# ViV99/slam-experiments

Measured on NVIDIA B200. Metric: hamming_pairs_per_sec, higher is better.
Workload: dtype u8

## Files before the change

slam_experiments_b200/csrc/hm_tc.cu:

```cuda
#include <math.h>
#include <stdlib.h>

#include <mutex>
#include <type_traits>

#include <cuda_fp16.h>

#include "hm_common.cuh"
#include "hm_tcgen05.cuh"

#ifndef HM_F4_TILE_N
#define HM_F4_TILE_N 128
#endif

namespace hm {

namespace {

constexpr int kRowBlock = 128;
constexpr int kMBlocks = 2;
constexpr int kBlockM = kRowBlock * kMBlocks;
constexpr int kSlabBytes = kRowBlock * 128;
constexpr int kPadRows = HM_PREPARED_TILE_ROWS;
constexpr int kTmemCols = 512;
constexpr uint32_t kSpinLimit = 1u << 26;

static_assert(kPadRows % kBlockM == 0, "prepared padding must cover whole query blocks");

struct CoreI8 {
    using Acc = int;
    static constexpr int kSlabs = 2;
    static constexpr int kRowBytes = HM_PREPARED_ROW_BYTES;
    static constexpr int kTileN = 128;
    static constexpr int kStages = 4;
    static constexpr int kUnits = 4;
    static constexpr int kColSplit = 1;
    static constexpr bool kRegisterHandover = false;
    static constexpr bool kScales = false;
    static constexpr int kPrologueTiles = 45;
    static __device__ __forceinline__ Acc lowest() { return INT_MIN; }
    static __device__ __forceinline__ Acc from_bits(uint32_t x) { return (int)x; }
    static __device__ __forceinline__ Acc max3(Acc a, Acc b, Acc c) { return __vimax3_s32(a, b, c); }
    static __device__ __forceinline__ Acc max2(Acc a, Acc b) { return max(a, b); }
    static __device__ __forceinline__ bool valid(Acc v) { return v >= -256; }
    static __device__ __forceinline__ unsigned distance(Acc v) { return (unsigned)((256 - v) >> 1); }
    static __device__ __forceinline__ unsigned encode(Acc v) { return (unsigned)(v + 257); }
    static __device__ __forceinline__ Acc floor_from(unsigned e) { return (int)e - 259; }
    static __device__ __forceinline__ uint32_t pack2(uint32_t lo, uint32_t hi) { return ((uint32_t)max((int)lo, -32768) & 0xFFFFu) | ((uint32_t)max((int)hi, -32768) << 16); }
    static __device__ __forceinline__ Acc unpack(uint32_t p, int hi) { return hi ? (int)p >> 16 : (int)(short)(p & 0xFFFFu); }
    static constexpr uint32_t kLowestBits = 0x80000000u;
};

struct CoreF4 {
    using Acc = float;
    static constexpr int kSlabs = 1;
    static constexpr int kRowBytes = HM_PREPARED_F4_ROW_BYTES;
    static constexpr int kTileN = HM_F4_TILE_N;
#ifndef HM_F4_STAGES
#define HM_F4_STAGES 6
#endif
    static constexpr int kStages = HM_F4_TILE_N == 96 ? 10 : HM_F4_TILE_N == 64 ? 14 : HM_F4_STAGES;
#ifndef HM_F4_UNITS
#define HM_F4_UNITS (HM_F4_TILE_N == 96 ? 5 : HM_F4_TILE_N == 64 ? 7 : 3)
#endif
    static constexpr int kUnits = HM_F4_UNITS;
    static constexpr int kColSplit = 2;
    static constexpr bool kRegisterHandover = true;
    static constexpr bool kScales = true;
    static constexpr int kPrologueTiles = 90;
    static __device__ __forceinline__ Acc lowest() { return -INFINITY; }
    static __device__ __forceinline__ Acc from_bits(uint32_t x) { return __uint_as_float(x); }
    static __device__ __forceinline__ Acc max3(Acc a, Acc b, Acc c) { return fmaxf(fmaxf(a, b), c); }
    static __device__ __forceinline__ Acc max2(Acc a, Acc b) { return fmaxf(a, b); }
    static __device__ __forceinline__ bool valid(Acc v) { return v >= -256.0f; }
    static __device__ __forceinline__ unsigned distance(Acc v) { return (unsigned)((256 - (int)v) >> 1); }
    static __device__ __forceinline__ unsigned encode(Acc v) { return (unsigned)((int)v + 257); }
    static __device__ __forceinline__ Acc floor_from(unsigned e) { return (float)((int)e - 259); }
    static __device__ __forceinline__ uint32_t pack2(uint32_t lo, uint32_t hi)
    {
        const __half2 h = __floats2half2_rn(__uint_as_float(lo), __uint_as_float(hi));
        return *reinterpret_cast<const uint32_t*>(&h);
    }
    static __device__ __forceinline__ Acc unpack(uint32_t p, int hi)
    {
        const __half2 h = *reinterpret_cast<const __half2*>(&p);
        return hi ? __high2float(h) : __low2float(h);
    }
    static constexpr uint32_t kLowestBits = 0xFF800000u;
};

template <class C> __host__ __device__ constexpr int row_block_bytes() { return kRowBlock * C::kRowBytes; }
template <class C> __host__ __device__ constexpr int a_bytes() { return kMBlocks * row_block_bytes<C>(); }
template <class C> __host__ __device__ constexpr int b_stage_bytes() { return C::kTileN * C::kRowBytes; }
template <class C> __host__ __device__ constexpr int epilogue_warps() { return 4 * kMBlocks * C::kColSplit; }
template <class C> __host__ __device__ constexpr int control_warps() { return C::kRegisterHandover ? 4 : 2; }
template <class C> __host__ __device__ constexpr int threads() { return 32 * (control_warps<C>() + epilogue_warps<C>()); }
constexpr int kHandoverBytes = kBlockM * 16;
constexpr int kBarrierBytes = 512;
template <class C> __host__ __device__ constexpr int smem_bytes() { return 1024 + a_bytes<C>() + C::kStages * b_stage_bytes<C>() + kBarrierBytes + kHandoverBytes; }
static_assert((2 * CoreF4::kStages + 1 + 2 * CoreF4::kUnits) * 8 + 16 <= kBarrierBytes, "barrier block");
static_assert((2 * CoreI8::kStages + 1 + 2 * CoreI8::kUnits) * 8 + 16 <= kBarrierBytes, "barrier block");
__host__ __device__ constexpr int ct_gcd(int a, int b) { return b == 0 ? a : ct_gcd(b, a % b); }
template <class C> __host__ __device__ constexpr int issuer_period() { return C::kStages / ct_gcd(C::kStages, C::kUnits) * C::kUnits; }
constexpr int kScaleCols = 32;
constexpr int kScaleCol = kTmemCols - kScaleCols;
static_assert(CoreF4::kUnits * CoreF4::kTileN <= kScaleCol, "accumulator units must end before the scale factors");

struct PrepareParams {
    const uint8_t* bits;
    long long n, stride, batch_stride;
    long long padded_rows;
    uint8_t* out;
};

__global__ void __launch_bounds__(256) hm_prepare_kernel(const PrepareParams P)
{
    const long long chunks_per_problem = P.padded_rows * 16;
    const long long o = (long long)blockIdx.x * blockDim.x + threadIdx.x;
    if (o >= chunks_per_problem) return;
    const int b = blockIdx.y;
    const long long rb = o >> 11;
    const int rem = (int)(o & 2047);
    const int slab = rem >> 10;
    const int rem2 = rem & 1023;
    const int rr = (rem2 >> 3) & 7;
    const int r = ((rem2 >> 6) << 3) | rr;
    const int c = (rem2 & 7) ^ rr;
    const long long row = rb * kRowBlock + r;
    uint4 v = make_uint4(0, 0, 0, 0);
    if (row < P.n) {
        const uint8_t* src = P.bits + (long long)b * P.batch_stride + row * P.stride + slab * 16 + c * 2;
        const unsigned bits16 = (unsigned)src[0] | ((unsigned)src[1] << 8);
        unsigned w[4];
#pragma unroll
        for (int i = 0; i < 4; ++i) {
            const unsigned nib = (bits16 >> (4 * i)) & 0xF;
            const unsigned spread = (nib & 1) | ((nib & 2) << 7) | ((nib & 4) << 14) | ((nib & 8) << 21);
            w[i] = (spread * 0xFEu) ^ 0xFFFFFFFFu;
        }
        v = make_uint4(w[0], w[1], w[2], w[3]);
    }
    uint4* dst = reinterpret_cast<uint4*>(P.out + (long long)b * P.padded_rows * HM_PREPARED_ROW_BYTES);
    dst[o] = v;
}

__device__ __forceinline__ uint4 expand_bits_e2m1(unsigned bits32)
{
    unsigned w[4];
#pragma unroll
    for (int i = 0; i < 4; ++i) {
        const unsigned by = (bits32 >> (8 * i)) & 0xFF;
        unsigned sgn = 0;
#pragma unroll
        for (int j = 0; j < 8; ++j) sgn |= ((by >> j) & 1u) << (4 * j + 3);
        w[i] = 0xAAAAAAAAu ^ sgn;
    }
    return make_uint4(w[0], w[1], w[2], w[3]);
}

__global__ void __launch_bounds__(256) hm_prepare_f4_kernel(const PrepareParams P)
{
    const long long chunks_per_problem = P.padded_rows * 8;
    const long long o = (long long)blockIdx.x * blockDim.x + threadIdx.x;
    if (o >= chunks_per_problem) return;
    const int b = blockIdx.y;
    const long long rb = o >> 10;
    const int rem = (int)(o & 1023);
    const int rr = (rem >> 3) & 7;
    const int r = ((rem >> 6) << 3) | rr;
    const int c = (rem & 7) ^ rr;
    const long long row = rb * kRowBlock + r;
    uint4 v = make_uint4(0, 0, 0, 0);
    if (row < P.n) {
        const unsigned bits32 = *reinterpret_cast<const unsigned*>(P.bits + (long long)b * P.batch_stride + row * P.stride + c * 4);
        v = expand_bits_e2m1(bits32);
    }
    uint4* dst = reinterpret_cast<uint4*>(P.out + (long long)b * P.padded_rows * HM_PREPARED_F4_ROW_BYTES);
    dst[o] = v;
}

struct TcParams {
    const uint8_t* qbits;
    long long q_bits_stride, q_bits_batch_stride;
    const int* q_index;
    long long q_index_batch_stride;
    const int* nq_dyn;
    const uint8_t* qprep;
    const uint8_t* tprep;
    long long nq, nt;
    long long q_padded, t_padded;
    int tiles_per_split;
    int ntiles;
    unsigned long long train_base;
    unsigned long long* out;
    long long out_split_stride;
    int* error_flag;
    unsigned long long* final_out;
    unsigned* counters;
    int splits;
    unsigned* row_floor;
    ExchangeArgs xch;
    long long q_blocks_valid;
    long long* clock_probe;
    SelectArgs sel;
    long long* trace;
    int trace_first;
};

#ifndef HM_TC_TRACE
#define HM_TC_TRACE 0
#endif
#ifndef HM_TC_EXPERIMENT
#define HM_TC_EXPERIMENT 0
#endif
#ifndef HM_ISSUER_LAST
#define HM_ISSUER_LAST 1
#endif
constexpr bool kIssuerLast = HM_ISSUER_LAST != 0;
#ifndef HM_COMMIT_MODE
#define HM_COMMIT_MODE 0
#endif
constexpr int kTraceTiles = 96;
constexpr int kTraceSlots = 8;
constexpr int kCtaSlots = 24;
__device__ __forceinline__ void cta_mark(const TcParams& P, int slot)
{
#if HM_TC_TRACE
    if (P.trace) {
        unsigned long long t;
        asm volatile("mov.u64 %0, %%globaltimer;" : "=l"(t));
        const long long cta = ((long long)blockIdx.z * gridDim.y + blockIdx.y) * gridDim.x + blockIdx.x;
        long long* rec = P.trace + kTraceTiles * kTraceSlots + cta * kCtaSlots;
        rec[slot] = (long long)t;
        rec[slot + 12] = clock64();
        if (slot == 0) {
            unsigned smid;
            asm volatile("mov.u32 %0, %%smid;" : "=r"(smid));
            rec[11] = smid;
        }
    }
#endif
}
__device__ __forceinline__ void trace_mark(const TcParams& P, int tile, int slot)
{
#if HM_TC_TRACE == 1
    tile -= P.trace_first;
    if (P.trace && blockIdx.x == 0 && blockIdx.y == 0 && blockIdx.z == 0 && tile >= 0 && tile < kTraceTiles)
        P.trace[tile * kTraceSlots + slot] = clock64();
#endif
}

template <class Acc>
struct Top2 {
    Acc v1, v2;
    unsigned i1, i2;
    uint32_t sa[4], sb[4];
    Acc f;
#if HM_TC_TRACE
    unsigned slow;
#endif
};

__device__ __forceinline__ void bounded_wait(uint64_t* bar, uint32_t parity, int* error_flag)
{
    uint32_t spins = 0;
    while (!ptx::mbar_try_wait(bar, parity)) {
        if (++spins > kSpinLimit) {
            if (error_flag) atomicExch(error_flag, 1);
            __trap();
        }
    }
}

__device__ __forceinline__ void bounded_wait_addr(uint32_t bar_addr, uint32_t parity, int* error_flag)
{
    uint32_t spins = 0;
    while (!ptx::mbar_try_wait_addr(bar_addr, parity)) {
        if (++spins > kSpinLimit) {
            if (error_flag) atomicExch(error_flag, 1);
            __trap();
        }
    }
}

#define HM_R8(a, o) "+r"(a[o]), "+r"(a[o + 1]), "+r"(a[o + 2]), "+r"(a[o + 3]), "+r"(a[o + 4]), "+r"(a[o + 5]), "+r"(a[o + 6]), "+r"(a[o + 7])
#define HM_R32(a) HM_R8(a, 0), HM_R8(a, 8), HM_R8(a, 16), HM_R8(a, 24)
__device__ __forceinline__ void tmem_ld_fence4(uint32_t (&a)[32], uint32_t (&b)[32], uint32_t (&c)[32], uint32_t (&d)[32])
{
    asm volatile("tcgen05.wait::ld.sync.aligned;\n" : HM_R32(a), HM_R32(b), HM_R32(c), HM_R32(d) : : "memory");
}
__device__ __forceinline__ void tmem_ld_fence48(uint32_t (&a)[32], uint32_t (&b)[16])
{
    asm volatile("tcgen05.wait::ld.sync.aligned;\n" : HM_R32(a), HM_R8(b, 0), HM_R8(b, 8) : : "memory");
}
__device__ __forceinline__ void tmem_ld_fence64(uint32_t (&a)[64])
{
    asm volatile("tcgen05.wait::ld.sync.aligned;\n" : HM_R8(a, 0), HM_R8(a, 8), HM_R8(a, 16), HM_R8(a, 24), HM_R8(a, 32), HM_R8(a, 40), HM_R8(a, 48), HM_R8(a, 56) : : "memory");
}

template <class C, int kMode, int kGroups = 4>
__device__ __forceinline__ void scan_chunk(const uint32_t* r, unsigned colbase, Top2<typename C::Acc>& s)
{
    using Acc = typename C::Acc;
    static_assert(kGroups == 2 || kGroups == 4 || kGroups == 8, "8-column groups per compare");
    Acc gm[kGroups];
#pragma unroll
    for (int g = 0; g < kGroups; ++g) {
        const int o = g * 8;
        gm[g] = C::max3(C::max3(C::from_bits(r[o]), C::from_bits(r[o + 1]), C::from_bits(r[o + 2])),
                        C::max3(C::from_bits(r[o + 3]), C::from_bits(r[o + 4]), C::from_bits(r[o + 5])),
                        C::max2(C::from_bits(r[o + 6]), C::from_bits(r[o + 7])));
    }
    Acc m;
    if constexpr (kGroups == 8) m = C::max3(C::max3(gm[0], gm[1], gm[2]), C::max3(gm[3], gm[4], gm[5]), C::max2(gm[6], gm[7]));
    else if constexpr (kGroups == 4) m = C::max3(gm[0], gm[1], C::max2(gm[2], gm[3]));
    else m = C::max2(gm[0], gm[1]);
    constexpr bool kFloor = kMode == 1, kTop1 = kMode == 2;
    if (m > (kFloor ? s.f : kTop1 ? s.v1 : s.v2)) {
#if HM_TC_TRACE
        s.slow += 1;
#endif
#pragma unroll
        for (int g = 0; g < kGroups; ++g) {
            const Acc x = gm[g];
            if (x > (kFloor ? s.f : kTop1 ? s.v1 : s.v2)) {
                const int o = g * 8;
                const uint32_t p0 = C::pack2(r[o], r[o + 1]), p1 = C::pack2(r[o + 2], r[o + 3]);
                const uint32_t p2 = C::pack2(r[o + 4], r[o + 5]), p3 = C::pack2(r[o + 6], r[o + 7]);
                const unsigned idx = colbase + o;
                if (kTop1 || x > s.v1) {
                    if (!kTop1) {
                        s.v2 = s.v1; s.i2 = s.i1;
                        s.sb[0] = s.sa[0]; s.sb[1] = s.sa[1]; s.sb[2] = s.sa[2]; s.sb[3] = s.sa[3];
                    }
                    s.v1 = x; s.i1 = idx;
                    s.sa[0] = p0; s.sa[1] = p1; s.sa[2] = p2; s.sa[3] = p3;
                } else {
                    s.v2 = x; s.i2 = idx;
                    s.sb[0] = p0; s.sb[1] = p1; s.sb[2] = p2; s.sb[3] = p3;
                }
                if (kFloor) s.f = C::max2(s.v2, s.f);
            }
        }
    }
}

template <class C, int kN>
__device__ __forceinline__ void mask_tail(uint32_t* r, unsigned colbase, unsigned limit)
{
    if (colbase + kN > limit) {
#pragma unroll
        for (int j = 0; j < kN; ++j)
            if (colbase + j >= limit) r[j] = C::kLowestBits;
    }
}

#ifndef HM_ARRIVE_ELECT
#define HM_ARRIVE_ELECT 1
#endif
#ifndef HM_SCAN_FLAT64
#define HM_SCAN_FLAT64 1
#endif
#ifndef HM_FLOOR_DENSE_TILES
#define HM_FLOOR_DENSE_TILES 32
#endif
#ifndef HM_FLOOR_LATE_MASK
#define HM_FLOOR_LATE_MASK 15
#endif

#ifndef HM_F4_A_TMEM
#define HM_F4_A_TMEM 0
#endif
constexpr int kATmemCol = 384;
constexpr int kATmemColsPerBlock = 32;

template <class C>
__device__ __forceinline__ void issue_half(int h, uint32_t a_block, uint32_t b_stage, uint32_t tmem_d, uint32_t idesc,
                                           uint32_t tmem_sf)
{
    constexpr int kHalf = C::kSlabs * 2;
#pragma unroll
    for (int jj = 0; jj < kHalf; ++jj) {
        const int j = h * kHalf + jj;
        const int slab = j >> 2, k = j & 3;
        const uint64_t db = ptx::kmajor_sw128_desc_from_lo(b_stage + ((slab * kSlabBytes + k * 32) >> 4));
        if constexpr (C::kScales && HM_F4_A_TMEM) {
            ptx::mma_mxf4_ts(tmem_d, a_block + 8 * j, db, idesc, tmem_sf, tmem_sf + kScaleCols / 2, j != 0);
        } else {
            const uint64_t da = ptx::kmajor_sw128_desc_from_lo(a_block + ((slab * kSlabBytes + k * 32) >> 4));
            if constexpr (C::kScales) ptx::mma_mxf4_ss(tmem_d, da, db, idesc, tmem_sf, tmem_sf + kScaleCols / 2, j != 0);
            else                      ptx::mma_i8_ss(tmem_d, da, db, idesc, j != 0);
        }
    }
}

template <class C, int kMode>
__device__ __forceinline__ void tc_knn2_body(const TcParams& P)
{
    constexpr bool kFloor = kMode == 1;
    using Acc = typename C::Acc;
    constexpr int kStages = C::kStages;
    constexpr int kUnits = C::kUnits;
    constexpr int kABytes = a_bytes<C>();
    constexpr int kBStageBytes = b_stage_bytes<C>();
    constexpr int kRowBlockBytes = row_block_bytes<C>();
    constexpr int kTileN = C::kTileN;

    extern __shared__ uint8_t smem_raw[];
    uint8_t* smem = smem_raw + ((1024u - (ptx::smem_u32(smem_raw) & 1023u)) & 1023u);
    uint8_t* smem_a = smem;
    uint8_t* smem_b = smem + kABytes;
    uint64_t* bars = reinterpret_cast<uint64_t*>(smem + kABytes + kStages * kBStageBytes);
    uint64_t* full_bar = bars;
    uint64_t* empty_bar = bars + kStages;
    uint64_t* a_full_bar = bars + 2 * kStages;
    uint64_t* tmem_full_bar = bars + 2 * kStages + 1;
    uint64_t* tmem_empty_bar = tmem_full_bar + kUnits;
    uint32_t* tmem_base_slot = reinterpret_cast<uint32_t*>(tmem_empty_bar + kUnits);
    uint32_t* smem_base_slot = tmem_base_slot + 2;
    ulonglong2* handover = reinterpret_cast<ulonglong2*>(smem + kABytes + kStages * kBStageBytes + kBarrierBytes);

    const int warp = __shfl_sync(0xffffffffu, threadIdx.x >> 5, 0);
    const int lane = threadIdx.x & 31;
    if (threadIdx.x == 0) cta_mark(P, 0);
    if (threadIdx.x == 0 && (blockIdx.x | blockIdx.y | blockIdx.z) == 0 && P.clock_probe) {
        unsigned long long t;
        asm volatile("mov.u64 %0, %%globaltimer;" : "=l"(t));
        P.clock_probe[0] = (long long)t;
        P.clock_probe[1] = clock64();
    }
    const int qb = blockIdx.x;
    const int split = blockIdx.y;
    const int b = blockIdx.z;

    const uint32_t cs = ptx::cluster_nctarank();
    const uint32_t crank = ptx::cluster_ctarank();
    const uint16_t cmask = (uint16_t)((1u << cs) - 1);
    const bool has_a = qb < P.q_blocks_valid;
    auto rows_present = [&]() -> long long { return P.nq_dyn ? min((long long)__ldg(P.nq_dyn + b), P.nq) : P.nq; };
    if (P.nq_dyn && (long long)(qb - (int)crank) * kBlockM >= rows_present()) return;

    const int tile_begin = split * P.tiles_per_split;
    const int tile_end = min(tile_begin + P.tiles_per_split, P.ntiles);
    const int my_tiles = tile_end - tile_begin;

    constexpr int kProducerWarp = kIssuerLast ? epilogue_warps<C>() : 0;
    constexpr int kIssuerWarp = kIssuerLast ? epilogue_warps<C>() + 1 : 1;
    constexpr int kFirstEpiWarp = kIssuerLast ? 0 : 2;
    static_assert(kIssuerLast || !C::kRegisterHandover, "the control warps must form the last warpgroup");
    static_assert(!C::kRegisterHandover || (epilogue_warps<C>() == 16 && threads<C>() == 640),
                  "the register budget (4 x 32 + 16 x 112 = 20 x 96) assumes 20 warps launched at 96 registers");
    if (warp == kProducerWarp && lane == 0) {
        *smem_base_slot = ptx::smem_u32(smem);
        for (int i = 0; i < kStages; ++i) {
            ptx::mbar_init(&full_bar[i], 1);
            ptx::mbar_init(&empty_bar[i], cs);
        }
        ptx::mbar_init(a_full_bar, 1);
        for (int i = 0; i < kUnits; ++i) {
            ptx::mbar_init(&tmem_full_bar[i], 1);
            ptx::mbar_init(&tmem_empty_bar[i], 4 * C::kColSplit);
        }
        ptx::fence_barrier_init();
        ptx::fence_proxy_async();
    } else if (warp == kIssuerWarp) {
        ptx::tmem_alloc(tmem_base_slot, kTmemCols);
        ptx::tmem_relinquish();
    }
    ptx::tc_fence_before();
    if (cs > 1) ptx::cluster_sync();
    else __syncthreads();
    ptx::tc_fence_after();
    const uint32_t tmem_base = *tmem_base_slot;

    if constexpr (C::kScales) {
        if (warp >= kFirstEpiWarp && warp < kFirstEpiWarp + 4) {
            uint32_t ones[32];
#pragma unroll
            for (int i = 0; i < 32; ++i) ones[i] = 0x7F7F7F7Fu;
            const uint32_t taddr = tmem_base + ((uint32_t)((warp & 3) * 32) << 16) + kScaleCol;
            static_assert(kScaleCols == 32, "one x32 store per lane quarter");
            ptx::tmem_st_32x32(taddr, ones);
            ptx::tmem_st_wait();
        }
        if (HM_F4_A_TMEM) {
            static_assert(!HM_F4_A_TMEM || C::kUnits * C::kTileN <= kATmemCol, "accumulator units overlap the A operand");
            static_assert(!HM_F4_A_TMEM || kATmemCol + kMBlocks * kATmemColsPerBlock <= kScaleCol, "A operand overlaps the scale factors");
            if (warp >= kFirstEpiWarp && warp < kFirstEpiWarp + 4 * kMBlocks) {
                const int wq = warp & 3, wblk = ((warp - kFirstEpiWarp) >> 2) & 1;
                const int r = wq * 32 + lane;
                const long long qrow = (long long)qb * kBlockM + wblk * kRowBlock + r;
                uint32_t words[32];
#pragma unroll
                for (int i = 0; i < 32; ++i) words[i] = 0u;
                if (qrow < rows_present()) {
                    if (P.qbits) {
                        const int* qidx = P.q_index ? P.q_index + (long long)b * P.q_index_batch_stride : nullptr;
                        const long long srow = qidx ? (long long)__ldg(qidx + qrow) : qrow;
                        const uint4* src = reinterpret_cast<const uint4*>(P.qbits + (long long)b * P.q_bits_batch_stride + srow * P.q_bits_stride);
                        const uint4 lo = src[0], hi = src[1];
                        const unsigned bits[8] = {lo.x, lo.y, lo.z, lo.w, hi.x, hi.y, hi.z, hi.w};
#pragma unroll
                        for (int c = 0; c < 8; ++c) {
                            const uint4 v = expand_bits_e2m1(bits[c]);
                            words[4 * c] = v.x; words[4 * c + 1] = v.y; words[4 * c + 2] = v.z; words[4 * c + 3] = v.w;
                        }
                    } else if (has_a) {
                        const uint8_t* img = P.qprep + ((long long)b * P.q_padded + (long long)qb * kBlockM + wblk * kRowBlock) * C::kRowBytes;
                        const uint4* row = reinterpret_cast<const uint4*>(img + (r >> 3) * 1024 + (r & 7) * 128);
#pragma unroll
                        for (int c = 0; c < 8; ++c) {
                            const uint4 v = row[c ^ (r & 7)];
                            words[4 * c] = v.x; words[4 * c + 1] = v.y; words[4 * c + 2] = v.z; words[4 * c + 3] = v.w;
                        }
                    }
                }
                ptx::tmem_st_32x32(tmem_base + ((uint32_t)(wq * 32) << 16) + kATmemCol + wblk * kATmemColsPerBlock, words);
                ptx::tmem_st_wait();
            }
        } else if (P.qbits) {
            const uint8_t* qsrc = P.qbits + (long long)b * P.q_bits_batch_stride;
            const int* qidx = P.q_index ? P.q_index + (long long)b * P.q_index_batch_stride : nullptr;
            const long long nq_eff = rows_present();
            for (int o = threadIdx.x; o < kBlockM * 8; o += blockDim.x) {
                const int blk = o >> 10, rem = o & 1023;
                const int rr = (rem >> 3) & 7;
                const int r = ((rem >> 6) << 3) | rr;
                const int c = (rem & 7) ^ rr;
                const long long qrow = (long long)qb * kBlockM + blk * kRowBlock + r;
                uint4 v = make_uint4(0, 0, 0, 0);
                if (qrow < nq_eff) {
                    const long long srow = qidx ? (long long)__ldg(qidx + qrow) : qrow;
                    v = expand_bits_e2m1(*reinterpret_cast<const unsigned*>(qsrc + srow * P.q_bits_stride + c * 4));
                }
                reinterpret_cast<uint4*>(smem_a)[o] = v;
            }
            ptx::fence_proxy_async();
        }
        ptx::tc_fence_before();
        __syncthreads();
        ptx::tc_fence_after();
    }

    if (threadIdx.x == 0) cta_mark(P, 1);
    ulonglong2 my_keys = make_ulonglong2(kNoMatch, kNoMatch);
    long long my_row = -1;
    int my_row_in_cta = 0;

    auto run_producer = [&]() {
        if (lane == 0) {
            if (has_a && !P.qbits && !(C::kScales && HM_F4_A_TMEM)) {
                const uint8_t* qsrc = P.qprep + ((long long)b * P.q_padded + (long long)qb * kBlockM) * C::kRowBytes;
                ptx::mbar_arrive_expect_tx(a_full_bar, kABytes);
                ptx::bulk_g2s(smem_a, qsrc, kABytes, a_full_bar);
            }
            const uint8_t* tsrc = P.tprep + (long long)b * P.t_padded * C::kRowBytes;
            const uint32_t piece = kBStageBytes / cs;
            for (int i = 0; i < (HM_TC_EXPERIMENT >= 5 ? 0 : my_tiles); ++i) {
                const int stage = i % kStages;
                const uint32_t use = i / kStages;
#if HM_TC_EXPERIMENT < 4
                bounded_wait(&empty_bar[stage], (use & 1) ^ 1, P.error_flag);
#endif
                trace_mark(P, i, 0);
                ptx::mbar_arrive_expect_tx(&full_bar[stage], kBStageBytes);
                uint8_t* dst = smem_b + stage * kBStageBytes + crank * piece;
                const uint8_t* src = tsrc + (long long)(tile_begin + i) * kBStageBytes + crank * piece;
                if (cs > 1) ptx::bulk_g2s_multicast(dst, src, piece, &full_bar[stage], cmask);
                else        ptx::bulk_g2s(dst, src, piece, &full_bar[stage]);
            }
        }
    };
    auto run_issuer = [&]() {
        const bool leader = ptx::elect_one();
        const uint32_t idesc = C::kScales ? ptx::make_mxf4_idesc(kRowBlock, kTileN) : ptx::make_i8_idesc(kRowBlock, kTileN);
        constexpr bool kATmem = C::kScales && HM_F4_A_TMEM;
        const uint32_t a_addr = kATmem ? tmem_base + kATmemCol : ptx::smem_u32(smem_a) >> 4;
        constexpr uint32_t kABlockStep = kATmem ? (uint32_t)kATmemColsPerBlock : (uint32_t)(kRowBlockBytes >> 4);
        const uint32_t b_addr = ptx::smem_u32(smem_b) >> 4;
        const uint32_t tmem_sf = tmem_base + kScaleCol;
        if (has_a && !P.qbits && !(C::kScales && HM_F4_A_TMEM)) bounded_wait(a_full_bar, 0, P.error_flag);
        constexpr int kPeriod = issuer_period<C>();
        static_assert(kPeriod % kStages == 0 && (2 * kPeriod) % kUnits == 0 && ((2 * kPeriod / kUnits) & 1) == 0,
                      "unit parities must repeat with the period");
        uint32_t sphase = 0;
        bool ready0 = false;
        for (int base = 0; base < my_tiles; base += kPeriod) {
#pragma unroll
            for (int j = 0; j < kPeriod; ++j) {
                if (base + j < my_tiles) {
                    const int stage = j % kStages;
                    const uint32_t full_par = sphase ^ ((j / kStages) & 1);
                    const int unit_a = (2 * j) % kUnits, unit_b = (2 * j + 1) % kUnits;
                    const uint32_t par_a = (((2 * j) / kUnits) & 1) ^ 1, par_b = (((2 * j + 1) / kUnits) & 1) ^ 1;
                    const uint32_t b_stage = b_addr + stage * (kBStageBytes >> 4);
                    if (leader) trace_mark(P, base + j, 7);
                    if (!ready0) {
#if HM_TC_EXPERIMENT < 4
                        bounded_wait(&full_bar[stage], full_par, P.error_flag);
#endif
#if HM_TC_EXPERIMENT < 3
                        bounded_wait(&tmem_empty_bar[unit_a], par_a, P.error_flag);
#endif
                    }
                    if (leader) trace_mark(P, base + j, 1);
                    ptx::tc_fence_after();
                    if (leader) issue_half<C>(0, a_addr, b_stage, tmem_base + unit_a * kTileN, idesc, tmem_sf);
#if HM_TC_EXPERIMENT >= 3
                    const bool ready1 = true;
#else
                    const bool ready1 = __all_sync(0xffffffffu, ptx::mbar_test_wait(&tmem_empty_bar[unit_b], par_b));
#endif
                    if (leader) {
                        issue_half<C>(1, a_addr, b_stage, tmem_base + unit_a * kTileN, idesc, tmem_sf);
#if HM_TC_EXPERIMENT != 6 && HM_COMMIT_MODE == 0
                        ptx::tc_commit(&tmem_full_bar[unit_a]);
#endif
                    }
                    if (!ready1) bounded_wait(&tmem_empty_bar[unit_b], par_b, P.error_flag);
                    if (leader) trace_mark(P, base + j, 6);
                    ptx::tc_fence_after();
                    if (leader) issue_half<C>(0, a_addr + kABlockStep, b_stage, tmem_base + unit_b * kTileN, idesc, tmem_sf);
                    ready0 = false;
                    if (base + j + 1 < my_tiles) {
                        const int n = j + 1;
#if HM_TC_EXPERIMENT >= 4
                        ready0 = true;
#else
                        ready0 = __all_sync(0xffffffffu,
                                            ptx::mbar_test_wait(&full_bar[n % kStages], sphase ^ ((n / kStages) & 1))
#if HM_TC_EXPERIMENT < 3
                                            && ptx::mbar_test_wait(&tmem_empty_bar[(2 * n) % kUnits], (((2 * n) / kUnits) & 1) ^ 1)
#endif
                                            );
#endif
                    }
                    if (leader) {
                        issue_half<C>(1, a_addr + kABlockStep, b_stage, tmem_base + unit_b * kTileN, idesc, tmem_sf);
#if HM_TC_EXPERIMENT == 6 || HM_COMMIT_MODE == 1
                        ptx::tc_commit(&tmem_full_bar[unit_a]);
#endif
                        ptx::tc_commit(&tmem_full_bar[unit_b]);
                        if (cs > 1) ptx::tc_commit_multicast(&empty_bar[stage], cmask);
                        else        ptx::tc_commit(&empty_bar[stage]);
                    }
                }
            }
            sphase ^= (kPeriod / kStages) & 1;
        }
        __syncwarp();
    };
    auto run_epilogue = [&]() {
        constexpr int kCols = kTileN / C::kColSplit;
        const int quarter = warp & 3;
        const int mblk = ((warp - kFirstEpiWarp) >> 2) & 1;
        const int half = (warp - kFirstEpiWarp) >> 3;
        const int row_in_cta = mblk * kRowBlock + quarter * 32 + lane;
        const long long row = (long long)qb * kBlockM + row_in_cta;
        Top2<Acc> s;
        s.v1 = s.v2 = C::lowest();
        s.i1 = s.i2 = 0;
#pragma unroll
        for (int e = 0; e < 4; ++e) s.sa[e] = s.sb[e] = 0;
        s.f = C::floor_from(0);
#if HM_TC_TRACE
        s.slow = 0;
#endif
        unsigned floor_code = 0;
        const long long first_row = (long long)tile_begin * kTileN;
        const unsigned limit = (unsigned)min((long long)my_tiles * kTileN, P.nt - first_row);
        const uint32_t bars_addr = ptx::lds_volatile_u32(ptx::smem_u32(smem_base_slot)) + kABytes + kStages * kBStageBytes;
        const uint32_t unit_full_addr = bars_addr + (2 * kStages + 1) * 8;
        const uint32_t unit_empty_addr = unit_full_addr + kUnits * 8;
        int unit = mblk;
        uint32_t unit_use = 0;
        unsigned floor_pending = 0;
        auto refresh_floor = [&](int i) {
            if constexpr (kFloor) {
                if (i < HM_FLOOR_DENSE_TILES || (i & HM_FLOOR_LATE_MASK) == 0) {
                    floor_code = max(floor_code, floor_pending);
                    s.f = C::max2(s.f, C::floor_from(floor_code));
                    if (row < P.nq) {
                        unsigned* floor_ptr = P.row_floor + ((long long)b * P.nq + row);
                        const unsigned e = C::valid(s.v2) ? C::encode(s.v2) : 0u;
                        if (e > floor_code) { atomicMax(floor_ptr, e); floor_code = e; }
                        floor_pending = __ldcg(floor_ptr);
                    }
                }
            }
        };
        auto process_tile = [&](int i) {
            bounded_wait_addr(unit_full_addr + unit * 8, unit_use & 1, P.error_flag);
#if HM_TC_TRACE == 2
            if (warp == kFirstEpiWarp && lane == 0 && (i == 8 || i == 32 || i == 64 || i == 192)) cta_mark(P, i == 8 ? 5 : i == 32 ? 6 : i == 64 ? 7 : 8);
#endif
            if (warp == kFirstEpiWarp && lane == 0) trace_mark(P, i, 3);
            if (warp == kFirstEpiWarp + 7 && lane == 0) trace_mark(P, i, 5);
            ptx::tc_fence_after();
            const uint32_t taddr = tmem_base + ((uint32_t)(quarter * 32) << 16) + unit * kTileN + half * kCols;
            const unsigned colbase = (unsigned)i * kTileN + half * kCols;
            if constexpr (C::kColSplit == 1) {
                uint32_t r0[32], r1[32], r2[32], r3[32];
                ptx::tmem_ld_32x32(taddr, r0);
                ptx::tmem_ld_32x32(taddr + 32, r1);
                ptx::tmem_ld_32x32(taddr + 64, r2);
                ptx::tmem_ld_32x32(taddr + 96, r3);
                refresh_floor(i);
                tmem_ld_fence4(r0, r1, r2, r3);
                ptx::tc_fence_before();
                __syncwarp();
                if (HM_ARRIVE_ELECT ? ptx::elect_one() : lane == 0) ptx::mbar_arrive_addr(unit_empty_addr + unit * 8);
                if (colbase + kCols > limit) {
                    mask_tail<C, 32>(r0, colbase, limit);
                    mask_tail<C, 32>(r1, colbase + 32, limit);
                    mask_tail<C, 32>(r2, colbase + 64, limit);
                    mask_tail<C, 32>(r3, colbase + 96, limit);
                }
                scan_chunk<C, kMode>(r0, colbase, s);
                scan_chunk<C, kMode>(r1, colbase + 32, s);
                scan_chunk<C, kMode>(r2, colbase + 64, s);
                scan_chunk<C, kMode>(r3, colbase + 96, s);
            } else {
                if constexpr (kCols == 64) {
                    uint32_t r[64];
#if HM_TC_EXPERIMENT < 2
                    ptx::tmem_ld_32x64(taddr, r);
                    refresh_floor(i);
                    tmem_ld_fence64(r);
#endif
                    ptx::tc_fence_before();
                    __syncwarp();
                    if (HM_ARRIVE_ELECT ? ptx::elect_one() : lane == 0) ptx::mbar_arrive_addr(unit_empty_addr + unit * 8);
#if HM_TC_EXPERIMENT != 0
                    unit += 2;
                    if (unit >= kUnits) { unit -= kUnits; ++unit_use; }
                    return;
#endif
                    mask_tail<C, 64>(r, colbase, limit);
#if HM_SCAN_FLAT64
                    scan_chunk<C, kMode, 8>(r, colbase, s);
#else
                    scan_chunk<C, kMode>(r, colbase, s);
                    scan_chunk<C, kMode>(r + 32, colbase + 32, s);
#endif
                } else if constexpr (kCols == 32) {
                    uint32_t r[32];
                    ptx::tmem_ld_32x32(taddr, r);
                    refresh_floor(i);
                    asm volatile("tcgen05.wait::ld.sync.aligned;\n" : HM_R32(r) : : "memory");
                    ptx::tc_fence_before();
                    __syncwarp();
                    if (HM_ARRIVE_ELECT ? ptx::elect_one() : lane == 0) ptx::mbar_arrive_addr(unit_empty_addr + unit * 8);
                    mask_tail<C, 32>(r, colbase, limit);
                    scan_chunk<C, kMode>(r, colbase, s);
                } else {
                    static_assert(kCols == 64 || kCols == 48, "column split");
                    uint32_t r0[32], r1[16];
                    ptx::tmem_ld_32x32(taddr, r0);
                    ptx::tmem_ld_32x16(taddr + 32, r1);
                    refresh_floor(i);
                    tmem_ld_fence48(r0, r1);
                    ptx::tc_fence_before();
                    __syncwarp();
                    if (HM_ARRIVE_ELECT ? ptx::elect_one() : lane == 0) ptx::mbar_arrive_addr(unit_empty_addr + unit * 8);
                    mask_tail<C, 32>(r0, colbase, limit);
                    mask_tail<C, 16>(r1, colbase + 32, limit);
                    scan_chunk<C, kMode>(r0, colbase, s);
                    scan_chunk<C, kMode, 2>(r1, colbase + 32, s);
                }
            }
            unit += 2;
            if (unit >= kUnits) { unit -= kUnits; ++unit_use; }
            if (warp == kFirstEpiWarp && lane == 0) trace_mark(P, i, 4);
        };
#pragma unroll 1
        for (int i = 0; i < my_tiles; ++i) process_tile(i);
        if (warp == kFirstEpiWarp && lane == 0) cta_mark(P, 2);
#if HM_TC_TRACE
        if (P.trace) {
            const long long cta = ((long long)blockIdx.z * gridDim.y + blockIdx.y) * gridDim.x + blockIdx.x;
            long long* rec = P.trace + kTraceTiles * kTraceSlots + cta * kCtaSlots;
            const unsigned any = __reduce_max_sync(0xffffffffu, s.slow);
            const unsigned sum = __reduce_add_sync(0xffffffffu, s.slow);
            if (lane == 0) { atomicAdd((unsigned long long*)&rec[9], (unsigned long long)any); atomicAdd((unsigned long long*)&rec[10], (unsigned long long)sum); }
        }
#endif
        const unsigned long long gbase = P.train_base + (unsigned long long)first_row;
        auto fold_group = [&](Acc v, unsigned i0, const uint32_t (&p)[4]) {
            if (!C::valid(v)) return;
#pragma unroll
            for (int e = 0; e < 8; ++e) {
                const Acc x = C::unpack(p[e >> 1], e & 1);
                if (C::valid(x)) top2_insert(my_keys.x, my_keys.y, ((unsigned long long)C::distance(x) << 32) | (gbase + i0 + e));
            }
        };
        fold_group(s.v1, s.i1, s.sa);
        if (kMode != 2) fold_group(s.v2, s.i2, s.sb);
        else my_keys.y = kNoMatch;
        if (half == 1) handover[row_in_cta] = my_keys;
        else my_row = row;
        my_row_in_cta = row_in_cta;
    };

    auto run_tail = [&](auto worker_tag) {
        constexpr bool kWorker = decltype(worker_tag)::value;
        ptx::tc_fence_before();
        if (cs > 1) ptx::cluster_sync();
        else __syncthreads();
        if (kWorker && threadIdx.x == 0) cta_mark(P, 3);
        if (warp == kIssuerWarp) {
            ptx::tc_fence_after();
            ptx::tmem_dealloc(tmem_base, kTmemCols);
        }
        if (kWorker && my_row >= 0 && my_row < rows_present()) {
            if constexpr (C::kColSplit == 2) {
                const ulonglong2 o = handover[my_row_in_cta];
                top2_insert(my_keys.x, my_keys.y, o.x);
                top2_insert(my_keys.x, my_keys.y, o.y);
            }
            unsigned long long* out = P.out + (long long)split * P.out_split_stride + ((long long)b * P.nq + my_row) * 2;
            *reinterpret_cast<ulonglong2*>(out) = my_keys;
            if (!P.counters) select_candidate(P.sel, b, my_keys);
        }
        if (P.counters) {
            int* flag = reinterpret_cast<int*>(tmem_base_slot + 1);
            if (last_cta_arrives(&P.counters[(long long)b * gridDim.x + qb], (unsigned)P.splits, flag)) {
                const long long row = (long long)qb * kBlockM + threadIdx.x;
                const bool has_row = kWorker && threadIdx.x < kBlockM && row < rows_present();
                ulonglong2 k = make_ulonglong2(kNoMatch, kNoMatch);
                if (has_row) fold_partials(P.out, P.splits, P.out_split_stride, (long long)b * P.nq + row, k.x, k.y);
                if (P.xch.world > 1 && (long long)qb * kBlockM < P.nq) k = exchange_and_merge(P.xch, row, has_row, k, qb);
                if (has_row) {
                    *reinterpret_cast<ulonglong2*>(P.final_out + ((long long)b * P.nq + row) * 2) = k;
                    select_candidate(P.sel, b, k);
                }
            }
        }
        if (kWorker && threadIdx.x == 0) cta_mark(P, 4);
        if (kWorker && threadIdx.x == 0 && (blockIdx.x | blockIdx.y | blockIdx.z) == 0 && P.clock_probe) {
            unsigned long long t;
            asm volatile("mov.u64 %0, %%globaltimer;" : "=l"(t));
            P.clock_probe[2] = (long long)t;
            P.clock_probe[3] = clock64();
        }
    };

    if constexpr (C::kRegisterHandover) {
        if (warp >= kProducerWarp) {
            asm volatile("setmaxnreg.dec.sync.aligned.u32 32;\n");
            if (warp == kProducerWarp) run_producer();
            else if (warp == kIssuerWarp) run_issuer();
            run_tail(std::false_type{});
            return;
        }
        asm volatile("setmaxnreg.inc.sync.aligned.u32 112;\n");
        run_epilogue();
        run_tail(std::true_type{});
    } else {
        if (warp == kProducerWarp) run_producer();
        else if (warp == kIssuerWarp) run_issuer();
        else run_epilogue();
        run_tail(std::true_type{});
    }
}

__global__ void __launch_bounds__(threads<CoreI8>(), 1) hm_i8_knn2_kernel(const TcParams P) { tc_knn2_body<CoreI8, 0>(P); }
__global__ void __launch_bounds__(threads<CoreF4>(), 1) hm_f4_knn2_kernel(const TcParams P) { tc_knn2_body<CoreF4, 0>(P); }
__global__ void __launch_bounds__(threads<CoreI8>(), 1) hm_i8_knn2_floor_kernel(const TcParams P) { tc_knn2_body<CoreI8, 1>(P); }
__global__ void __launch_bounds__(threads<CoreF4>(), 1) hm_f4_knn2_floor_kernel(const TcParams P) { tc_knn2_body<CoreF4, 1>(P); }
__global__ void __launch_bounds__(threads<CoreI8>(), 1) hm_i8_knn1_kernel(const TcParams P) { tc_knn2_body<CoreI8, 2>(P); }
__global__ void __launch_bounds__(threads<CoreF4>(), 1) hm_f4_knn1_kernel(const TcParams P) { tc_knn2_body<CoreF4, 2>(P); }

using KernelFn = void (*)(const TcParams);
template <class C> KernelFn kernel_of(int mode = 0);
template <> KernelFn kernel_of<CoreI8>(int mode) { return mode == 1 ? hm_i8_knn2_floor_kernel : mode == 2 ? hm_i8_knn1_kernel : hm_i8_knn2_kernel; }
template <> KernelFn kernel_of<CoreF4>(int mode) { return mode == 1 ? hm_f4_knn2_floor_kernel : mode == 2 ? hm_f4_knn1_kernel : hm_f4_knn2_kernel; }

struct TcPlan {
    int ntiles, splits, tiles_per_split;
    int cluster;
    long long qblocks;
};

int floor_max_tiles()
{
    static int v = -1;
    if (v < 0) {
        const char* e = getenv("HM_FLOOR_MAX_TILES");
        v = e ? atoi(e) : 0x7fffffff;
    }
    return v;
}

int floor_min_tiles_unsplit()
{
    static int v = -1;
    if (v < 0) {
        const char* e = getenv("HM_FLOOR_MIN_TILES_UNSPLIT");
        v = e ? atoi(e) : 0x7fffffff;
    }
    return v;
}

int cluster_override()
{
    static int v = -1;
    if (v < 0) {
        const char* e = getenv("HM_I8_CLUSTER");
        v = e ? atoi(e) : 0;
        if (v != 1 && v != 2 && v != 4) v = 0;
    }
    return v;
}

constexpr int kMaxDevices = 64;
std::mutex g_launch_state_mu;

int current_device_slot()
{
    int dev = 0;
    if (cudaGetDevice(&dev) != cudaSuccess) { cudaGetLastError(); dev = 0; }
    return (dev >= 0 && dev < kMaxDevices) ? dev : -1;
}

template <class C>
cudaError_t ensure_smem_opt_in()
{
    static bool done[kMaxDevices] = {};
    const int dev = current_device_slot();
    std::lock_guard<std::mutex> lock(g_launch_state_mu);
    if (dev >= 0 && done[dev]) return cudaSuccess;
    for (int mode = 0; mode < 3; ++mode) {
        const cudaError_t e = cudaFuncSetAttribute(kernel_of<C>(mode), cudaFuncAttributeMaxDynamicSharedMemorySize, smem_bytes<C>());
        if (e != cudaSuccess) return e;
    }
    if (dev >= 0) done[dev] = true;
    return cudaSuccess;
}

template <class C>
int resident_ctas(int cs, int sm_count)
{
    static int cache[kMaxDevices][5] = {};
    if (cs <= 1) return sm_count;
    const int dev = current_device_slot();
    if (dev >= 0) {
        std::lock_guard<std::mutex> lock(g_launch_state_mu);
        if (cache[dev][cs]) return cache[dev][cs];
    }
    int v = sm_count;
    if (ensure_smem_opt_in<C>() == cudaSuccess) {
        cudaLaunchConfig_t cfg{};
        cfg.gridDim = dim3(cs * 64, 1, 1);
        cfg.blockDim = dim3(threads<C>());
        cfg.dynamicSmemBytes = smem_bytes<C>();
        cudaLaunchAttribute attr[1];
        attr[0].id = cudaLaunchAttributeClusterDimension;
        attr[0].val.clusterDim.x = (unsigned)cs;
        attr[0].val.clusterDim.y = 1;
        attr[0].val.clusterDim.z = 1;
        cfg.attrs = attr;
        cfg.numAttrs = 1;
        int n = 0;
        if (cudaOccupancyMaxActiveClusters(&n, kernel_of<C>(), &cfg) == cudaSuccess && n > 0) v = n * cs;
        else cudaGetLastError();
    } else {
        cudaGetLastError();
    }
    if (dev >= 0) {
        std::lock_guard<std::mutex> lock(g_launch_state_mu);
        cache[dev][cs] = v;
    }
    return v;
}

template <class C>
int prologue_tiles()
{
    static int v = -1;
    if (v < 0) {
        const char* e = getenv("HM_PROLOGUE_TILES");
        v = e ? atoi(e) : C::kPrologueTiles;
    }
    return v;
}

int cluster_min_tiles()
{
    static int v = -1;
    if (v < 0) {
        const char* e = getenv("HM_CLUSTER_MIN_TILES");
        v = e ? atoi(e) : 1024;
    }
    return v;
}

template <class C>
TcPlan plan_tc_cluster(long long nq, long long nt, int batch, int sm_count, int cluster)
{
    TcPlan pl{};
    const long long qb = ceil_div(nq, kBlockM);
    pl.cluster = cluster;
    pl.qblocks = ceil_div(qb, pl.cluster) * pl.cluster;
    sm_count = resident_ctas<C>(pl.cluster, sm_count);
    pl.ntiles = (int)ceil_div(nt, C::kTileN);
    const long long items = pl.qblocks * batch;
    long long best_cost = -1;
    int best = 1;
    const int max_splits = (int)min((long long)pl.ntiles, 4096ll);
    for (int s = 1; s <= max_splits; ++s) {
        const long long tps = ceil_div(pl.ntiles, s);
        const long long real_s = ceil_div(pl.ntiles, tps);
        const long long waves = ceil_div(items * real_s, sm_count);
        const long long cost = waves * (tps + prologue_tiles<C>());
        if (best_cost < 0 || cost < best_cost) {
            best_cost = cost;
            best = s;
        }
        if (items * s > 16ll * sm_count) break;
    }
    pl.tiles_per_split = (int)ceil_div(pl.ntiles, best);
    pl.splits = (int)ceil_div(pl.ntiles, pl.tiles_per_split);
    return pl;
}

template <class C>
TcPlan plan_tc(long long nq, long long nt, int batch, int sm_count)
{
    if (cluster_override()) return plan_tc_cluster<C>(nq, nt, batch, sm_count, cluster_override());
    if (ceil_div(nq, kBlockM) >= 2) {
        const TcPlan pl = plan_tc_cluster<C>(nq, nt, batch, sm_count, 2);
        if (pl.tiles_per_split >= cluster_min_tiles()) return pl;
    }
    return plan_tc_cluster<C>(nq, nt, batch, sm_count, 1);
}

template <class C>
long long padded_rows(long long n) { return ceil_div(ceil_div(n, C::kTileN) * C::kTileN, kPadRows) * kPadRows; }

template <class C>
size_t partials_bytes(long long nq, long long nt, int batch, int sm_count)
{
    const TcPlan pl = plan_tc<C>(nq, nt, batch, sm_count);
    return (size_t)pl.splits * batch * nq * 2 * sizeof(unsigned long long);
}

inline size_t zeroed_bytes(long long row_blocks, long long rows) { return counters_bytes(row_blocks) + counters_bytes((rows + 1) / 2 * 2); }

template <class C>
size_t workspace_bytes_of(long long nq, long long nt, int batch, int sm_count, bool with_prepare)
{
    size_t b = 256 + zeroed_bytes(plan_tc<C>(nq, nt, batch, sm_count).qblocks * batch, nq * batch) + partials_bytes<C>(nq, nt, batch, sm_count);
    b = (b + 1023) & ~(size_t)1023;
    if (with_prepare) b += (size_t)(padded_rows<C>(nq) + padded_rows<C>(nt)) * C::kRowBytes * batch;
    return b;
}

template <class C>
int launch_prepared(const void* qprep, long long nq, const void* tprep, long long nt, int batch,
                    unsigned long long train_base, unsigned long long* out, void* ws, size_t ws_bytes,
                    int sm_count, cudaStream_t stream, const unsigned long long** out_partials,
                    int* out_groups, const ExchangeArgs* exchange, bool top1 = false, const QueryBits* qbits = nullptr,
                    const SelectArgs* select = nullptr)
{
    HM_CUDA_CHECK(ensure_smem_opt_in<C>());
    const TcPlan pl = plan_tc<C>(nq, nt, batch, sm_count);
    if ((long long)pl.ntiles * C::kTileN > (1ll << 32)) {
        set_error("train set too large for 32-bit trainIdx");
        return HM_ERR_UNSUPPORTED;
    }
    const bool keep_partials = out == nullptr;
    const size_t cbytes = zeroed_bytes(pl.qblocks * batch, nq * batch);
    const size_t need = 256 + cbytes + partials_bytes<C>(nq, nt, batch, sm_count);
    if (!ws || ws_bytes < need) {
        set_error("workspace too small: need %zu bytes, got %zu", need, ws_bytes);
        return HM_ERR_WORKSPACE;
    }
    TcParams P{};
    if (qbits && qbits->bits) {
// ... 289 lines not shown
```

Before: 13900.

## Unroll epilogue steady state over TMEM units and use three-input max

```diff
diff --git a/slam_experiments_b200/csrc/hm_tc.cu b/slam_experiments_b200/csrc/hm_tc.cu
--- a/slam_experiments_b200/csrc/hm_tc.cu
+++ b/slam_experiments_b200/csrc/hm_tc.cu
@@ -70,7 +70,12 @@
     static constexpr int kPrologueTiles = 90;
     static __device__ __forceinline__ Acc lowest() { return -INFINITY; }
     static __device__ __forceinline__ Acc from_bits(uint32_t x) { return __uint_as_float(x); }
-    static __device__ __forceinline__ Acc max3(Acc a, Acc b, Acc c) { return fmaxf(fmaxf(a, b), c); }
+    static __device__ __forceinline__ Acc max3(Acc a, Acc b, Acc c)
+    {
+        float d;
+        asm("max.f32 %0, %1, %2, %3;" : "=f"(d) : "f"(a), "f"(b), "f"(c));
+        return d;
+    }
     static __device__ __forceinline__ Acc max2(Acc a, Acc b) { return fmaxf(a, b); }
     static __device__ __forceinline__ bool valid(Acc v) { return v >= -256.0f; }
     static __device__ __forceinline__ unsigned distance(Acc v) { return (unsigned)((256 - (int)v) >> 1); }
@@ -298,23 +303,35 @@
     asm volatile("tcgen05.wait::ld.sync.aligned;\n" : HM_R8(a, 0), HM_R8(a, 8), HM_R8(a, 16), HM_R8(a, 24), HM_R8(a, 32), HM_R8(a, 40), HM_R8(a, 48), HM_R8(a, 56) : : "memory");
 }
 
+template <class C, int N>
+__device__ __forceinline__ typename C::Acc max_tree(const typename C::Acc (&v)[N])
+{
+    if constexpr (N == 1) return v[0];
+    else if constexpr (N == 2) return C::max2(v[0], v[1]);
+    else {
+        typename C::Acc w[N / 3 + N % 3];
+#pragma unroll
+        for (int k = 0; k < N / 3; ++k) w[k] = C::max3(v[3 * k], v[3 * k + 1], v[3 * k + 2]);
+#pragma unroll
+        for (int k = 0; k < N % 3; ++k) w[N / 3 + k] = v[3 * (N / 3) + k];
+        return max_tree<C, N / 3 + N % 3>(w);
+    }
+}
+
 template <class C, int kMode, int kGroups = 4>
 __device__ __forceinline__ void scan_chunk(const uint32_t* r, unsigned colbase, Top2<typename C::Acc>& s)
 {
     using Acc = typename C::Acc;
     static_assert(kGroups == 2 || kGroups == 4 || kGroups == 8, "8-column groups per compare");
-    Acc gm[kGroups];
+    Acc part[2 * kGroups];
 #pragma unroll
     for (int g = 0; g < kGroups; ++g) {
         const int o = g * 8;
-        gm[g] = C::max3(C::max3(C::from_bits(r[o]), C::from_bits(r[o + 1]), C::from_bits(r[o + 2])),
-                        C::max3(C::from_bits(r[o + 3]), C::from_bits(r[o + 4]), C::from_bits(r[o + 5])),
-                        C::max2(C::from_bits(r[o + 6]), C::from_bits(r[o + 7])));
-    }
-    Acc m;
-    if constexpr (kGroups == 8) m = C::max3(C::max3(gm[0], gm[1], gm[2]), C::max3(gm[3], gm[4], gm[5]), C::max2(gm[6], gm[7]));
-    else if constexpr (kGroups == 4) m = C::max3(gm[0], gm[1], C::max2(gm[2], gm[3]));
-    else m = C::max2(gm[0], gm[1]);
+        part[2 * g] = C::max3(C::from_bits(r[o]), C::from_bits(r[o + 1]), C::from_bits(r[o + 2]));
+        part[2 * g + 1] = C::max3(C::max3(C::from_bits(r[o + 3]), C::from_bits(r[o + 4]), C::from_bits(r[o + 5])),
+                                  C::from_bits(r[o + 6]), C::from_bits(r[o + 7]));
+    }
+    const Acc m = max_tree<C, 2 * kGroups>(part);
     constexpr bool kFloor = kMode == 1, kTop1 = kMode == 2;
     if (m > (kFloor ? s.f : kTop1 ? s.v1 : s.v2)) {
 #if HM_TC_TRACE
@@ -322,7 +339,7 @@
 #endif
 #pragma unroll
         for (int g = 0; g < kGroups; ++g) {
-            const Acc x = gm[g];
+            const Acc x = C::max2(part[2 * g], part[2 * g + 1]);
             if (x > (kFloor ? s.f : kTop1 ? s.v1 : s.v2)) {
                 const int o = g * 8;
                 const uint32_t p0 = C::pack2(r[o], r[o + 1]), p1 = C::pack2(r[o + 2], r[o + 3]);
@@ -357,9 +374,6 @@
 
 #ifndef HM_ARRIVE_ELECT
 #define HM_ARRIVE_ELECT 1
-#endif
-#ifndef HM_SCAN_FLAT64
-#define HM_SCAN_FLAT64 1
 #endif
 #ifndef HM_FLOOR_DENSE_TILES
 #define HM_FLOOR_DENSE_TILES 32
@@ -672,32 +686,36 @@
         const uint32_t bars_addr = ptx::lds_volatile_u32(ptx::smem_u32(smem_base_slot)) + kABytes + kStages * kBStageBytes;
         const uint32_t unit_full_addr = bars_addr + (2 * kStages + 1) * 8;
         const uint32_t unit_empty_addr = unit_full_addr + kUnits * 8;
-        int unit = mblk;
-        uint32_t unit_use = 0;
+        const uint32_t tmem_warp = tmem_base + ((uint32_t)(quarter * 32) << 16) + half * kCols;
         unsigned floor_pending = 0;
-        auto refresh_floor = [&](int i) {
+        auto refresh_floor = [&]() {
             if constexpr (kFloor) {
-                if (i < HM_FLOOR_DENSE_TILES || (i & HM_FLOOR_LATE_MASK) == 0) {
-                    floor_code = max(floor_code, floor_pending);
-                    s.f = C::max2(s.f, C::floor_from(floor_code));
-                    if (row < P.nq) {
-                        unsigned* floor_ptr = P.row_floor + ((long long)b * P.nq + row);
-                        const unsigned e = C::valid(s.v2) ? C::encode(s.v2) : 0u;
-                        if (e > floor_code) { atomicMax(floor_ptr, e); floor_code = e; }
-                        floor_pending = __ldcg(floor_ptr);
-                    }
+                floor_code = max(floor_code, floor_pending);
+                s.f = C::max2(s.f, C::floor_from(floor_code));
+                if (row < P.nq) {
+                    unsigned* floor_ptr = P.row_floor + ((long long)b * P.nq + row);
+                    const unsigned e = C::valid(s.v2) ? C::encode(s.v2) : 0u;
+                    if (e > floor_code) { atomicMax(floor_ptr, e); floor_code = e; }
+                    floor_pending = __ldcg(floor_ptr);
                 }
             }
         };
-        auto process_tile = [&](int i) {
-            bounded_wait_addr(unit_full_addr + unit * 8, unit_use & 1, P.error_flag);
+        auto mark_complete = [&](int i) {
 #if HM_TC_TRACE == 2
             if (warp == kFirstEpiWarp && lane == 0 && (i == 8 || i == 32 || i == 64 || i == 192)) cta_mark(P, i == 8 ? 5 : i == 32 ? 6 : i == 64 ? 7 : 8);
 #endif
             if (warp == kFirstEpiWarp && lane == 0) trace_mark(P, i, 3);
             if (warp == kFirstEpiWarp + 7 && lane == 0) trace_mark(P, i, 5);
+        };
+        auto process_tile = [&](int i) {
+            const int unit = (2 * i + mblk) % kUnits;
+            bounded_wait_addr(unit_full_addr + unit * 8, ((2 * i + mblk) / kUnits) & 1, P.error_flag);
+            mark_complete(i);
             ptx::tc_fence_after();
-            const uint32_t taddr = tmem_base + ((uint32_t)(quarter * 32) << 16) + unit * kTileN + half * kCols;
+            auto refresh_floor_due = [&]() {
+                if (i < HM_FLOOR_DENSE_TILES || (i & HM_FLOOR_LATE_MASK) == 0) refresh_floor();
+            };
+            const uint32_t taddr = tmem_warp + unit * kTileN;
             const unsigned colbase = (unsigned)i * kTileN + half * kCols;
             if constexpr (C::kColSplit == 1) {
                 uint32_t r0[32], r1[32], r2[32], r3[32];
@@ -705,7 +723,7 @@
                 ptx::tmem_ld_32x32(taddr + 32, r1);
                 ptx::tmem_ld_32x32(taddr + 64, r2);
                 ptx::tmem_ld_32x32(taddr + 96, r3);
-                refresh_floor(i);
+                refresh_floor_due();
                 tmem_ld_fence4(r0, r1, r2, r3);
                 ptx::tc_fence_before();
                 __syncwarp();
@@ -725,28 +743,21 @@
                     uint32_t r[64];
 #if HM_TC_EXPERIMENT < 2
                     ptx::tmem_ld_32x64(taddr, r);
-                    refresh_floor(i);
+                    refresh_floor_due();
                     tmem_ld_fence64(r);
 #endif
                     ptx::tc_fence_before();
                     __syncwarp();
                     if (HM_ARRIVE_ELECT ? ptx::elect_one() : lane == 0) ptx::mbar_arrive_addr(unit_empty_addr + unit * 8);
 #if HM_TC_EXPERIMENT != 0
-                    unit += 2;
-                    if (unit >= kUnits) { unit -= kUnits; ++unit_use; }
                     return;
 #endif
                     mask_tail<C, 64>(r, colbase, limit);
-#if HM_SCAN_FLAT64
                     scan_chunk<C, kMode, 8>(r, colbase, s);
-#else
-                    scan_chunk<C, kMode>(r, colbase, s);
-                    scan_chunk<C, kMode>(r + 32, colbase + 32, s);
-#endif
                 } else if constexpr (kCols == 32) {
                     uint32_t r[32];
                     ptx::tmem_ld_32x32(taddr, r);
-                    refresh_floor(i);
+                    refresh_floor_due();
                     asm volatile("tcgen05.wait::ld.sync.aligned;\n" : HM_R32(r) : : "memory");
                     ptx::tc_fence_before();
                     __syncwarp();
@@ -758,7 +769,7 @@
                     uint32_t r0[32], r1[16];
                     ptx::tmem_ld_32x32(taddr, r0);
                     ptx::tmem_ld_32x16(taddr + 32, r1);
-                    refresh_floor(i);
+                    refresh_floor_due();
                     tmem_ld_fence48(r0, r1);
                     ptx::tc_fence_before();
                     __syncwarp();
@@ -769,12 +780,50 @@
                     scan_chunk<C, kMode, 2>(r1, colbase + 32, s);
                 }
             }
-            unit += 2;
-            if (unit >= kUnits) { unit -= kUnits; ++unit_use; }
             if (warp == kFirstEpiWarp && lane == 0) trace_mark(P, i, 4);
         };
+        int i = 0;
+        if constexpr (kCols == 64) {
+            constexpr int kDense = (HM_FLOOR_DENSE_TILES + kUnits - 1) / kUnits * kUnits;
+            constexpr int kRefreshPeriods = (HM_FLOOR_LATE_MASK + kUnits) / kUnits;
+            const int last = my_tiles - 1;
 #pragma unroll 1
-        for (int i = 0; i < my_tiles; ++i) process_tile(i);
+            for (; i < min(kDense, last); ++i) process_tile(i);
+            auto steady = [&](auto mblk_tag) {
+                constexpr int kMblk = decltype(mblk_tag)::value;
+#pragma unroll 1
+                while (i + kUnits <= last) {
+                    refresh_floor();
+                    const int periods = min(kRefreshPeriods, (last - i) / kUnits);
+#pragma unroll 1
+                    for (int p = 0; p < periods; ++p, i += kUnits) {
+#pragma unroll
+                        for (int j = 0; j < kUnits; ++j) {
+                            const int unit = (2 * j + kMblk) % kUnits;
+                            bounded_wait_addr(unit_full_addr + unit * 8, ((2 * j + kMblk) / kUnits) & 1, P.error_flag);
+                            mark_complete(i + j);
+                            ptx::tc_fence_after();
+                            uint32_t r[64];
+#if HM_TC_EXPERIMENT < 2
+                            ptx::tmem_ld_32x64(tmem_warp + unit * kTileN, r);
+                            tmem_ld_fence64(r);
+#endif
+                            ptx::tc_fence_before();
+                            __syncwarp();
+                            if (HM_ARRIVE_ELECT ? ptx::elect_one() : lane == 0) ptx::mbar_arrive_addr(unit_empty_addr + unit * 8);
+#if HM_TC_EXPERIMENT == 0
+                            scan_chunk<C, kMode, 8>(r, (unsigned)(i + j) * kTileN + half * kCols, s);
+#endif
+                            if (warp == kFirstEpiWarp && lane == 0) trace_mark(P, i + j, 4);
+                        }
+                    }
+                }
+            };
+            if (mblk == 0) steady(std::integral_constant<int, 0>{});
+            else           steady(std::integral_constant<int, 1>{});
+        }
+#pragma unroll 1
+        for (; i < my_tiles; ++i) process_tile(i);
         if (warp == kFirstEpiWarp && lane == 0) cta_mark(P, 2);
 #if HM_TC_TRACE
         if (P.trace) {
```

New measurement: 14000 (median of 6 runs). Within noise of the previous version (+0.7%).
